# AutonomousVehicleLaboratory/vision_semantic_segmentation

Measured on AMD Instinct MI355X. Metric: fused frames/sec/GPU (1920x1080 + 120k pts) + max|dlog-odds| vs ref, higher is better.
Workload: dtype f16 hi+lo split, MX-FP4 correction passes, fp32 accumulate

## Files before the change

### vision_semantic_segmentation_amd/csrc/seg_gemm.hip

```cpp
#include <cstdlib>
#include <cstring>
#include <type_traits>

#include "seg_types.h"

namespace avl {
namespace {

struct GemmArgs {
    const void* A;
    const void* W;
    const float* bias;
    const void* R;
    void* C;
    int lda, ldr, ldc;
    int M, N, K;
    int relu, out_f32;
    int ntiles;
    int nsub;
    long long a_lo_delta;
    const void* R_lo;
    void* C_lo;
};

// ... 429 lines not shown
                    Vec8<H>::store(cp + 8, hi);
                    if constexpr (IO != 0) {
                        if (csplit) {
#pragma unroll
                            for (int i = 0; i < 8; ++i) { lo[i] = v[i] - (float)(H)v[i]; hi[i] = v[8 + i] - (float)(H)v[8 + i]; }
                            H* cl = c_lo + (long long)m * ldc + cbase;
                            Vec8<H>::store(cl, lo);
                            Vec8<H>::store(cl + 8, hi);
                        }
                    }
                }
            }
        }
        if (t + nwg < total) init_acc(t + nwg);
    }
}

template <typename H, int WM, int WN, int MI, int STAGES, int NSUB, int IO, int AST, bool EXT>
int launch_ring_t(const GemmArgs& a0, int M, hipStream_t s, const RingExt& x) {
    constexpr int BM = WM * MI * 16, BN = WN * 64, LDS = (AST * BM + STAGES * BN) * 128;
    static_assert(LDS <= 160 * 1024, "ring does not fit LDS");
    AVL_HIP_CHECK(hipFuncSetAttribute(reinterpret_cast<const void*>(&k_gemm_ring<H, WM, WN, MI, STAGES, NSUB, IO, AST, EXT>),
                                      hipFuncAttributeMaxDynamicSharedMemorySize, LDS));
    GemmArgs a = a0;
    a.ntiles = (a.N + BN - 1) / BN;
    const int mtiles = (M + BM - 1) / BM;
    const int total = mtiles * a.ntiles;
    const int grid = total < 256 ? total : 256;
    hipLaunchKernelGGL((k_gemm_ring<H, WM, WN, MI, STAGES, NSUB, IO, AST, EXT>), dim3(grid), dim3(WM * WN * 64), LDS, s, a, mtiles, x);
    AVL_LAUNCH_CHECK();
    return AVL_OK;
}

template <typename H, int WM, int WN, int MI, int STAGES, int NSUB = 1, int IO = 0, int AST = STAGES>
int launch_ring(const GemmArgs& a, int M, hipStream_t s, const RingExt* x = nullptr) {
    if (x) return launch_ring_t<H, WM, WN, MI, STAGES, NSUB, IO, AST, true>(a, M, s, *x);
    return launch_ring_t<H, WM, WN, MI, STAGES, NSUB, IO, AST, false>(a, M, s, RingExt{});
}

template <typename T, int WM, int WN>
int launch_cfg(const GemmArgs& a, int mtiles, hipStream_t s) {
    constexpr int LDS = 2 * (WM * 64 + WN * 64) * 128;
    AVL_HIP_CHECK(hipFuncSetAttribute(reinterpret_cast<const void*>(&k_gemm<T, WM, WN>),
                                      hipFuncAttributeMaxDynamicSharedMemorySize, LDS));
    hipLaunchKernelGGL((k_gemm<T, WM, WN>), dim3(mtiles * a.ntiles), dim3(WM * WN * 64), LDS, s, a);
    AVL_LAUNCH_CHECK();
    return AVL_OK;
}

struct MxArgs {
    GemmArgs g;
    const char* Aq[2];
    const char* As[2];
    const char* Wq[2];
    const char* Ws[2];
    int ldaq;
    long long a_srows, w_srows;
    char* Cq[2];
    char* Cs[2];
    int ldcq;
    long long c_srows;
    int nmx;
    const char* Rq;
    const char* Rs;
    int ldrq;
    long long r_srows;
    int nmb1;
    const void* A2;
    int lda2, ldaq2;
    const char* Aq2[2];
    const char* As2[2];
    long long a_srows2;
    int stagger;
};

template <int IO, int MI>
__device__ __forceinline__ void mx_epilogue(const MxArgs& q, f32x4 (&acc)[MI][4], int nt, int mt, int wm, int wn, int fr, int kq) {
    typedef f16 H;
    typedef typename Half16<H>::v8 v8;
    constexpr int BM = 2 * MI * 16, BN = 256;
    const GemmArgs& p = q.g;
    const int nbase = nt * BN + wn * 64 + kq * 16;
    const bool ncol_ok = nbase + 16 <= p.N;
    const bool rsplit = p.R_lo != nullptr, csplit = p.C_lo != nullptr;
    const unsigned m0 = (unsigned)(mt * BM + wm * (MI * 16) + fr);
    const unsigned sc_r = (unsigned)(nbase >> 8) * (unsigned)q.r_srows * 8u + (unsigned)((nbase >> 5) & 7);
    const unsigned sc_c = (unsigned)(nbase >> 8) * (unsigned)q.c_srows * 8u + (unsigned)((nbase >> 5) & 7);
    v8 nr0 = {}, nr1 = {};
    uint2 npk = make_uint2(0u, 0u);
    unsigned nsb = 127u;
    auto load_res = [&](int mi) {
        const unsigned m = m0 + mi * 16;
        if (p.R && (int)m < p.M && ncol_ok) {
            const H* rp = static_cast<const H*>(p.R) + (m * (unsigned)p.ldr + (unsigned)nbase);
            nr0 = *reinterpret_cast<const v8*>(rp);
            nr1 = *reinterpret_cast<const v8*>(rp + 8);
            if (q.Rq) {
                npk = *reinterpret_cast<const uint2*>(q.Rq + (m * (unsigned)q.ldrq + (unsigned)(nbase / 2)));
                nsb = (unsigned char)q.Rs[sc_r + m * 8u];
            }
        }
    };
    load_res(0);
#pragma unroll
    for (int mi = 0; mi < MI; ++mi) {
        const unsigned m = m0 + mi * 16;
        const bool live = (int)m < p.M && ncol_ok;
        const v8 r0 = nr0, r1 = nr1;
        const uint2 pk = npk;
        const unsigned sb = nsb;
        if (mi + 1 < MI) load_res(mi + 1);
        float v[16];
#pragma unroll
        for (int nj = 0; nj < 4; ++nj)
#pragma unroll
            for (int r = 0; r < 4; ++r) v[nj * 4 + r] = acc[mi][nj][r];
        if (p.R && live) {
            float rl[16];
#pragma unroll
            for (int i = 0; i < 16; ++i) rl[i] = 0.f;
            if (rsplit) {
                const H* rlp = static_cast<const H*>(p.R_lo) + (m * (unsigned)p.ldr + (unsigned)nbase);
                const v8 l0 = *reinterpret_cast<const v8*>(rlp), l1 = *reinterpret_cast<const v8*>(rlp + 8);
#pragma unroll
                for (int i = 0; i < 8; ++i) { rl[i] = (float)l0[i]; rl[8 + i] = (float)l1[i]; }
            } else if (q.Rq) {
                typedef float v2f __attribute__((ext_vector_type(2)));
                const float sc = __uint_as_float(sb << 23);
#define AVL_FP4_DEC(w, sel, o) { const v2f d = __builtin_amdgcn_cvt_scalef32_pk_f32_fp4(w, sc, sel); rl[o] = d.x; rl[o + 1] = d.y; }
                AVL_FP4_DEC(pk.x, 0, 0) AVL_FP4_DEC(pk.x, 1, 2) AVL_FP4_DEC(pk.x, 2, 4) AVL_FP4_DEC(pk.x, 3, 6)
                AVL_FP4_DEC(pk.y, 0, 8) AVL_FP4_DEC(pk.y, 1, 10) AVL_FP4_DEC(pk.y, 2, 12) AVL_FP4_DEC(pk.y, 3, 14)
#undef AVL_FP4_DEC
            }
#pragma unroll
            for (int i = 0; i < 8; ++i) { v[i] += (float)r0[i] + rl[i]; v[8 + i] += (float)r1[i] + rl[8 + i]; }
        }
        if (p.relu) {
#pragma unroll
            for (int i = 0; i < 16; ++i) v[i] = fmaxf(v[i], 0.f);
        }
        v8 h0, h1;
#pragma unroll
        for (int i = 0; i < 8; ++i) { h0[i] = (H)v[i]; h1[i] = (H)v[8 + i]; }
        float hi[16], lo[16];
#pragma unroll
        for (int i = 0; i < 8; ++i) {
            hi[i] = (float)h0[i];
            hi[8 + i] = (float)h1[i];
            lo[i] = v[i] - hi[i];
            lo[8 + i] = v[8 + i] - hi[8 + i];
        }
        const unsigned coff = m * (unsigned)p.ldc + (unsigned)nbase;
        if (live) {
            H* cp = static_cast<H*>(p.C) + coff;
            *reinterpret_cast<v8*>(cp) = h0;
            *reinterpret_cast<v8*>(cp + 8) = h1;
        }
        if (csplit) {
            v8 l0, l1;
#pragma unroll
            for (int i = 0; i < 8; ++i) { l0[i] = (H)lo[i]; l1[i] = (H)lo[8 + i]; }
            if (live) {
                H* cl = static_cast<H*>(p.C_lo) + coff;
                *reinterpret_cast<v8*>(cl) = l0;
                *reinterpret_cast<v8*>(cl + 8) = l1;
            }
#pragma unroll
            for (int i = 0; i < 8; ++i) { lo[i] = (float)l0[i]; lo[8 + i] = (float)l1[i]; }
        }
        if constexpr (IO != 0) {
#pragma unroll
            for (int pl = 0; pl < 2; ++pl) {
                if (q.Cq[pl] == nullptr) continue;
                unsigned pq[2];
                const unsigned sq = quantize_fp4_block(pl == 0 ? hi : lo, pq);
                if (live) {
                    *reinterpret_cast<uint2*>(q.Cq[pl] + (m * (unsigned)q.ldcq + (unsigned)(nbase / 2))) = make_uint2(pq[0], pq[1]);
                    if ((kq & 1) == 0) q.Cs[pl][sc_c + m * 8u] = (char)sq;
                }
            }
        }
    }
}

template <int IO, int MI>
__global__ void __launch_bounds__(512) k_gemm_ring_mx(MxArgs q, int mtiles) {
    typedef f16 H;
    typedef typename Half16<H>::v8 v8;
    typedef int v8i __attribute__((ext_vector_type(8)));
    constexpr int WM = 2, WN = 4, STAGES = 2;
    constexpr int NW = WM * WN, BM = WM * MI * 16, BN = WN * 64;
    constexpr int A_BYTES = BM * 128, W_BYTES = BN * 128;
    constexpr int W_REGION = STAGES * A_BYTES, S_REGION = W_REGION + STAGES * W_BYTES;
    constexpr int S_BYTES = 4096;
    constexpr int A_INSTR = BM / 8 / NW, W_INSTR = BN / 8 / NW;
    extern __shared__ __attribute__((aligned(16))) char lds[];
    const GemmArgs& p = q.g;

    const int tid = threadIdx.x, lane = tid & 63;
    const int wave = __builtin_amdgcn_readfirstlane(tid >> 6);
    const int wm = wave / WN, wn = wave % WN;
    const int nwg = gridDim.x;
    int vb;
    {
        const int bid = blockIdx.x, xcd = bid & 7, local = bid >> 3, qq = nwg >> 3, r = nwg & 7;
        vb = (xcd < r ? xcd * (qq + 1) : r * (qq + 1) + (xcd - r) * qq) + local;
    }
    const int total = mtiles * p.ntiles;
    const int nmb = p.K / 256;
    const int nsub = 4 + q.nmx;
    const unsigned lds_base = lds_addr(lds);

    const int srow = lane >> 3, schunk = lane & 7;
    const unsigned ct = (unsigned)((schunk ^ srow) << 4);
    const unsigned a_lane16 = (unsigned)srow * (unsigned)(p.lda * 2) + ct, a_laneq = (unsigned)srow * (unsigned)q.ldaq + ct;
    const unsigned a_lane16_2 = (unsigned)srow * (unsigned)(q.lda2 * 2) + ct, a_laneq_2 = (unsigned)srow * (unsigned)q.ldaq2 + ct;
    unsigned w_off16[W_INSTR], w_offq[W_INSTR];
#pragma unroll
    for (int i = 0; i < W_INSTR; ++i) {
        const int r = (i * NW + wave) * 8 + srow;
        const int key = ((r >> 1) & 1) | (((r >> 4) & 3) << 1);
        w_off16[i] = (unsigned)r * (unsigned)(p.K * 2) + ((schunk ^ key) << 4);
        w_offq[i] = (unsigned)r * (unsigned)(p.K / 2) + ((schunk ^ key) << 4);
    }
    int pt = vb, pmb = 0, pj = 0, issued = 0;
    auto issue = [&]() {
        const int nt = pt % p.ntiles, mt = pt / p.ntiles;
        const unsigned abase = lds_base + (issued % STAGES) * A_BYTES + wave * 1024;
        const unsigned wbase = lds_base + W_REGION + (issued % STAGES) * W_BYTES + wave * 1024;
        const bool second = pmb >= q.nmb1;
        const int mbl = second ? pmb - q.nmb1 : pmb;
        if (pj < 4) {
            const long long rowb = second ? (long long)q.lda2 * 2 : (long long)p.lda * 2;
            const char* sa = static_cast<const char*>(second ? q.A2 : p.A) + ((long long)mt * BM + wave * 8) * rowb + (long long)(mbl * 4 + pj) * 128;
            const char* sw = static_cast<const char*>(p.W) + (long long)nt * BN * p.K * 2 + (long long)(pmb * 4 + pj) * 128;
            const unsigned al = second ? a_lane16_2 : a_lane16;
#pragma unroll
            for (int i = 0; i < A_INSTR; ++i) glds16_saddr(sa + (long long)i * (NW * 8) * rowb, al, abase + i * NW * 1024);
#pragma unroll
            for (int i = 0; i < W_INSTR; ++i) glds16_saddr(sw, w_off16[i], wbase + i * NW * 1024);
        } else {
            const int t = pj - 4;
            const long long rowb = second ? q.ldaq2 : q.ldaq;
            const char* sa = (second ? q.Aq2[t] : q.Aq[t]) + ((long long)mt * BM + wave * 8) * rowb + (long long)mbl * 128;
            const char* sw = q.Wq[t] + (long long)nt * BN * (p.K / 2) + (long long)pmb * 128;
            const unsigned al = second ? a_laneq_2 : a_laneq;
#pragma unroll
            for (int i = 0; i < A_INSTR; ++i) glds16_saddr(sa + (long long)i * (NW * 8) * rowb, al, abase + i * NW * 1024);
#pragma unroll
            for (int i = 0; i < W_INSTR; ++i) glds16_saddr(sw, w_offq[i], wbase + i * NW * 1024);
            if (wave < 4 && (wave >= 2 || wave * 128 < BM)) {
                const char* as = second ? q.As2[t] + ((long long)mbl * q.a_srows2 + (long long)mt * BM) * 8
                                        : q.As[t] + ((long long)mbl * q.a_srows + (long long)mt * BM) * 8;
                const char* ss = wave < 2 ? as + wave * 1024
                                          : q.Ws[t] + ((long long)pmb * q.w_srows + (long long)nt * BN) * 8 + (wave - 2) * 1024;
                glds16_saddr(ss, (unsigned)lane * 16u, lds_base + S_REGION + (issued % STAGES) * S_BYTES + wave * 1024);
// ... 58 lines not shown
                }
            }
            for (int u = 0; u < q.nmx; ++u, ++g) {
                asm volatile("s_waitcnt vmcnt(0)" ::: "memory");
                __builtin_amdgcn_s_barrier();
                const char* abase = lds + (g % STAGES) * A_BYTES + a_row0 * 128;
                const char* wbase = lds + (g % STAGES) * W_BYTES;
                const char* sbase = lds + (g % STAGES) * S_BYTES + S_REGION;
#pragma unroll
                for (int kk = 0; kk < 2; ++kk) {
                    if (kk == late && pt < total) issue();
                    int4 wf[4];
                    int ws[4];
#pragma unroll
                    for (int nj = 0; nj < 4; ++nj) {
                        wf[nj] = *reinterpret_cast<const int4*>(wbase + w_off[nj] + (((kk * 4 + kq) ^ w_key[nj]) << 4));
                        {
                            const uint2 w8 = *reinterpret_cast<const uint2*>(sbase + 2048 + (wn * 4 + (fr >> 2)) * 128 + ((fr & 3) * 4 + kq) * 8);
                            ws[nj] = (int)(((nj < 2 ? w8.x : w8.y) >> (8 * ((nj & 1) * 2 + kk))) & 0xffu);
                        }
                    }
                    const int achunk = ((kk * 4 + kq) ^ a_key) << 4;
                    int4 af = *reinterpret_cast<const int4*>(abase + achunk);
                    unsigned asw = *reinterpret_cast<const unsigned*>(sbase + a_row0 * 8 + kk * 4);
#pragma unroll
                    for (int mi = 0; mi < MI; ++mi) {
                        const int4 cur = af;
                        const int as = (int)((asw >> (8 * kq)) & 0xffu);
                        if (mi + 1 < MI) {
                            af = *reinterpret_cast<const int4*>(abase + (mi + 1) * 2048 + achunk);
                            asw = *reinterpret_cast<const unsigned*>(sbase + (a_row0 + (mi + 1) * 16) * 8 + kk * 4);
                        }
                        const v8i xa = {cur.x, cur.y, cur.z, cur.w, 0, 0, 0, 0};
#pragma unroll
                        for (int nj = 0; nj < 4; ++nj) {
                            const v8i wa = {wf[nj].x, wf[nj].y, wf[nj].z, wf[nj].w, 0, 0, 0, 0};
                            acc[mi][nj] = __builtin_amdgcn_mfma_scale_f32_16x16x128_f8f6f4(wa, xa, acc[mi][nj], 4, 4, 0, ws[nj], 0, as);
                        }
                    }
                }
            }
        }
        mx_epilogue<IO, MI>(q, acc, nt, mt, wm, wn, fr, kq);
        if (t + nwg < total) init_acc(t + nwg);
    }
}

template <int IO, int MI, int LATE>
__global__ void __launch_bounds__(512) k_gemm_mx_pipe(MxArgs q, int mtiles) {
    typedef f16 H;
    typedef typename Half16<H>::v8 v8;
    typedef int v8i __attribute__((ext_vector_type(8)));
    constexpr int WM = 2, WN = 4, STAGES = 2;
    constexpr int NW = WM * WN, BM = WM * MI * 16, BN = WN * 64;
    constexpr int A_BYTES = BM * 128, W_BYTES = BN * 128;
    constexpr int W_REGION = STAGES * A_BYTES, S_REGION = W_REGION + STAGES * W_BYTES;
    constexpr int S_BYTES = 4096;
    constexpr int A_INSTR = BM / 8 / NW, W_INSTR = BN / 8 / NW;
    constexpr int NS = 2 * MI, D = 3, EV = NS - D;
    constexpr int EW = MI == 8 ? 5 : EV;
    extern __shared__ __attribute__((aligned(16))) char lds[];
    const GemmArgs& p = q.g;

    const int tid = threadIdx.x, lane = tid & 63;
    const int wave = __builtin_amdgcn_readfirstlane(tid >> 6);
    const int wm = wave / WN, wn = wave % WN;
    const int nwg = gridDim.x;
    int vb;
    {
        const int bid = blockIdx.x, xcd = bid & 7, local = bid >> 3, qq = nwg >> 3, r = nwg & 7;
        vb = (xcd < r ? xcd * (qq + 1) : r * (qq + 1) + (xcd - r) * qq) + local;
    }
    const int ntiles = p.ntiles, nmx = q.nmx;
    const int total = mtiles * ntiles;
    const int nmb = p.K / 256;
    const int nsub = 4 + nmx;
    const unsigned lds_base = lds_addr(lds);

    auto lane_now = [&]() __attribute__((always_inline)) {
        unsigned l;
        asm volatile("v_mbcnt_lo_u32_b32 %0, -1, 0\n\tv_mbcnt_hi_u32_b32 %0, -1, %0" : "=v"(l));
        return l;
    };
    int pt = vb, pmb = 0, pj = 0, issued = 0, pmbl = 0;
    long long cur_rowb16 = 0, cur_rowbq = 0, cur_asrows = 0;
    const char *cur_a16 = nullptr, *cur_aq = nullptr, *cur_as = nullptr, *cur_w16 = nullptr, *cur_wq = nullptr, *cur_ws = nullptr;
    long long cur_aps = 0, cur_wps = 0;
    int p_mt = 0;
    auto set_input = [&](bool second) __attribute__((always_inline)) {
        const long long rows0 = (long long)p_mt * BM + wave * 8;
        if (!second) {
            cur_rowb16 = (long long)p.lda * 2; cur_rowbq = q.ldaq; cur_asrows = q.a_srows;
            cur_a16 = static_cast<const char*>(p.A) + rows0 * cur_rowb16;
            cur_aq = q.Aq[0] + rows0 * cur_rowbq;
            cur_as = q.As[0] + (long long)p_mt * BM * 8;
            cur_aps = q.Aq[1] - q.Aq[0];
        } else {
            cur_rowb16 = (long long)q.lda2 * 2; cur_rowbq = q.ldaq2; cur_asrows = q.a_srows2;
            cur_a16 = static_cast<const char*>(q.A2) + rows0 * cur_rowb16;
            cur_aq = q.Aq2[0] + rows0 * cur_rowbq;
            cur_as = q.As2[0] + (long long)p_mt * BM * 8;
            cur_aps = q.Aq2[1] - q.Aq2[0];
        }
        pmbl = 0;
    };
    auto set_tile = [&]() __attribute__((always_inline)) {
        const int nt_ = pt % ntiles;
        p_mt = pt / ntiles;
        cur_w16 = static_cast<const char*>(p.W) + (long long)nt_ * BN * p.K * 2;
        cur_wq = q.Wq[0] + (long long)nt_ * BN * (p.K / 2);
        cur_ws = q.Ws[0] + (long long)nt_ * BN * 8;
        cur_wps = q.Wq[1] - q.Wq[0];
        set_input(false);
    };
    auto issue_w = [&]() __attribute__((always_inline)) {
        const unsigned wbase = lds_base + W_REGION + (issued & 1) * W_BYTES + wave * 1024;
        const unsigned l = lane_now(), srow = l >> 3, cw = ((l & 7u) ^ (((srow >> 1) & 1u) | (((unsigned)(wave >> 1) & 3u) << 1))) << 4;
        const unsigned wr0 = (unsigned)wave * 8u + srow;
        if (pj < 4) {
            const char* sw = cur_w16 + (long long)(pmb * 4 + pj) * 128;
            const unsigned wl = wr0 * (unsigned)(p.K * 2) + cw;
#pragma unroll
            for (int i = 0; i < W_INSTR; ++i)
                glds16_saddr(sw + (long long)i * (NW * 8) * p.K * 2, wl, wbase + i * NW * 1024);
        } else {
            const char* sw = cur_wq + (pj == 4 ? 0 : cur_wps) + (long long)pmb * 128;
            const unsigned wl = wr0 * (unsigned)(p.K / 2) + cw;
#pragma unroll
            for (int i = 0; i < W_INSTR; ++i)
                glds16_saddr(sw + (long long)i * (NW * 8) * (p.K / 2), wl, wbase + i * NW * 1024);
        }
    };
    auto issue_a = [&]() __attribute__((always_inline)) {
        const unsigned abase = lds_base + (issued & 1) * A_BYTES + wave * 1024;
        const unsigned l = lane_now(), srow = l >> 3, ct = ((l & 7u) ^ srow) << 4;
        if (pj < 4) {
            const char* sa = cur_a16 + (long long)(pmbl * 4 + pj) * 128;
            const unsigned al = srow * (unsigned)cur_rowb16 + ct;
#pragma unroll
            for (int i = 0; i < A_INSTR; ++i)
                glds16_saddr(sa + (long long)i * (NW * 8) * cur_rowb16, al, abase + i * NW * 1024);
        } else {
            const long long ta = pj == 4 ? 0 : cur_aps, tw = pj == 4 ? 0 : cur_wps;
            const char* sa = cur_aq + ta + (long long)pmbl * 128;
            const unsigned a_lq = srow * (unsigned)cur_rowbq + ct;
#pragma unroll
            for (int i = 0; i < A_INSTR; ++i)
                glds16_saddr(sa + (long long)i * (NW * 8) * cur_rowbq, a_lq, abase + i * NW * 1024);
            if (wave < 4 && (wave >= 2 || wave * 128 < BM)) {
                const char* ss = wave < 2 ? cur_as + ta + (long long)pmbl * cur_asrows * 8 + wave * 1024
                                          : cur_ws + tw + (long long)pmb * q.w_srows * 8 + (wave - 2) * 1024;
                glds16_saddr(ss, l * 16u, lds_base + S_REGION + (issued & 1) * S_BYTES + wave * 1024);
            }
        }
        ++issued;
        if (++pj == nsub) {
            pj = 0;
            ++pmbl;
            if (++pmb == nmb) {
                pmb = 0;
                pt += nwg;
                if (pt < total) set_tile();
            } else if (pmb == q.nmb1) set_input(true);
        }
    };
    if (pt < total) set_tile();
    static_assert(NW == 8, "the DMA stagger assumes waves w and w + 4 on one SIMD");
    const bool early = wave >= 4 || q.stagger == 0;
    if (pt < total) { issue_w(); issue_a(); }
    if (pt < total) { issue_w(); issue_a(); }

    const int fr = lane & 15, kq = lane >> 4;
    const int a_row0 = wm * (MI * 16) + fr;
    const int wrow0 = wn * 64 + (fr >> 2) * 16 + (fr & 3);
    const int wkey_r = ((wrow0 >> 1) & 1) | (((wrow0 >> 4) & 3) << 1);
    const unsigned a_v0 = (unsigned)(a_row0 * 128 + ((kq ^ (a_row0 & 7)) << 4));
    const unsigned w_v0 = (unsigned)(W_REGION + wrow0 * 128 + ((kq ^ wkey_r) << 4));
    const unsigned sa_v = (unsigned)(S_REGION + a_row0 * 8 + kq);
    const unsigned sw_v = (unsigned)(S_REGION + 2048 + (wn * 4 + (fr >> 2)) * 128 + ((fr & 3) * 4 + kq) * 8);

    f32x4 acc[MI][4];
    auto init_acc = [&](int t) {
        const int nb = (t % ntiles) * BN + wn * 64 + kq * 16;
#pragma unroll
        for (int nj = 0; nj < 4; ++nj) {
            const float4 b = *reinterpret_cast<const float4*>(p.bias + nb + 4 * nj);
#pragma unroll
            for (int mi = 0; mi < MI; ++mi) acc[mi][nj] = f32x4{b.x, b.y, b.z, b.w};
        }
    };
    if (vb < total) init_acc(vb);

    int4 Af[NS], Wf[2][4];
    unsigned As[NS];
    uint2 Wsc = make_uint2(0u, 0u), Wsn = make_uint2(0u, 0u);
    auto rdA = [&](const char* slot, int kk, int mi) { return *reinterpret_cast<const int4*>(slot + (a_v0 ^ (unsigned)(kk * 64)) + mi * 2048); };
    auto rdW = [&](const char* slot, int kk, int nj) { return *reinterpret_cast<const int4*>(slot + (w_v0 ^ (unsigned)(kk * 64)) + nj * 512); };
    auto rdAs = [&](const char* slot, int kk, int mi) { return (unsigned)*reinterpret_cast<const unsigned char*>(slot + sa_v + mi * 128 + kk * 4); };
    auto rdWs = [&](const char* slot) { return *reinterpret_cast<const uint2*>(slot + sw_v); };

    int g = 0;
    bool w_sent = false;
    auto step = [&](auto kind_c, auto s_c, const bool next_q) __attribute__((always_inline)) {
        constexpr int KIND = decltype(kind_c)::value, S = decltype(s_c)::value;
        constexpr int kk = S / MI, mi = S % MI;
        const char* ab = lds + (g & 1) * A_BYTES;
        const char* wb = lds + (g & 1) * W_BYTES;
        const char* sb = lds + (g & 1) * S_BYTES;
        const char* abn = lds + ((g + 1) & 1) * A_BYTES;
        const char* wbn = lds + ((g + 1) & 1) * W_BYTES;
        const char* sbn = lds + ((g + 1) & 1) * S_BYTES;
        auto readA = [&](int t) {
            Af[t] = rdA(ab, t / MI, t % MI);
            if (KIND == 1) As[t] = rdAs(sb, t / MI, t % MI);
        };
        auto readAn = [&](int t) {
            Af[t] = rdA(abn, t / MI, t % MI);
            As[t] = rdAs(sbn, t / MI, t % MI);
        };
        if (EW != EV && S == EW) {
            if (LATE == 0 && !early && g > 0 && pt < total) issue_a();
            if (KIND == 0) asm volatile("s_waitcnt lgkmcnt(1)\n\ts_barrier" ::: "memory");
            else asm volatile("s_waitcnt lgkmcnt(2)\n\ts_barrier" ::: "memory");
            __builtin_amdgcn_sched_barrier(0);
            if (early && pt < total) { issue_w(); w_sent = true; }
        }
        if (EW != EV && LATE != 0 && !early && S == EW + LATE && pt < total) {
            issue_w();
            w_sent = true;
        }
        if (S == EV) {
            if (EW != EV && LATE == 0 && !early && pt < total) {
                issue_w();
                w_sent = true;
            }
            if (EW != EV && w_sent) asm volatile("s_waitcnt vmcnt(%0)\n\ts_waitcnt lgkmcnt(0)\n\ts_barrier" ::"n"(W_INSTR) : "memory");
            else asm volatile("s_waitcnt vmcnt(0)\n\ts_waitcnt lgkmcnt(0)\n\ts_barrier" ::: "memory");
            w_sent = false;
            __builtin_amdgcn_sched_barrier(0);
            if (early && pt < total) { if (EW == EV) issue_w(); issue_a(); }
#pragma unroll
            for (int nj = 0; nj < 4; ++nj) Wf[0][nj] = rdW(wbn, 0, nj);
            Wsn = rdWs(sbn);
            readAn(0);
        }
        if (!early && (EW == EV || LATE != 0) && S == EV + LATE && pt < total) {
            if (EW == EV) issue_w();
            issue_a();
        }
        if (S + D < NS) readA(S + D);
        if (S >= EV && S + 1 < NS) readAn(S - EV + 1);
        if constexpr (MI == 8 && S < 4) Wf[1][S] = rdW(wb, 1, S);
        if constexpr (MI == 4 && S < 2) { Wf[1][2 * S] = rdW(wb, 1, 2 * S); Wf[1][2 * S + 1] = rdW(wb, 1, 2 * S + 1); }
        if (KIND == 0) {
            const v8 af = __builtin_bit_cast(v8, Af[S]);
#pragma unroll
            for (int nj = 0; nj < 4; ++nj) acc[mi][nj] = Half16<H>::mfma(__builtin_bit_cast(v8, Wf[kk][nj]), af, acc[mi][nj]);
        } else {
            const v8i xa = {Af[S].x, Af[S].y, Af[S].z, Af[S].w, 0, 0, 0, 0};
            const int as = (int)As[S];
#define AVL_QMFMA(NJ)                                                                                                              \
    do {                                                                                                                           \
        const v8i wa = {Wf[kk][NJ].x, Wf[kk][NJ].y, Wf[kk][NJ].z, Wf[kk][NJ].w, 0, 0, 0, 0};                                       \
        const int ws = (int)((NJ) < 2 ? Wsc.x : Wsc.y);                                                                            \
        acc[mi][NJ] = __builtin_amdgcn_mfma_scale_f32_16x16x128_f8f6f4(wa, xa, acc[mi][NJ], 4, 4, ((NJ) & 1) * 2 + kk, ws, 0, as);      \
    } while (0)
            AVL_QMFMA(0); AVL_QMFMA(1); AVL_QMFMA(2); AVL_QMFMA(3);
#undef AVL_QMFMA
        }
        __builtin_amdgcn_sched_barrier(0);
    };
    auto substep = [&](auto kind_c, const bool next_q) __attribute__((always_inline)) {
#define AVL_STEP(N) step(kind_c, std::integral_constant<int, N>(), next_q)
        AVL_STEP(0); AVL_STEP(1); AVL_STEP(2); AVL_STEP(3); AVL_STEP(4); AVL_STEP(5); AVL_STEP(6); AVL_STEP(7);
        if constexpr (NS == 16) { AVL_STEP(8); AVL_STEP(9); AVL_STEP(10); AVL_STEP(11); AVL_STEP(12); AVL_STEP(13); AVL_STEP(14); AVL_STEP(15); }
#undef AVL_STEP
        Wsc = Wsn;
        ++g;
    };
    typedef std::integral_constant<int, 0> F16;
    typedef std::integral_constant<int, 1> FP4;

    asm volatile("s_waitcnt vmcnt(0)" ::: "memory");
    __builtin_amdgcn_s_barrier();
    for (int t = vb; t < total; t += nwg) {
        const int nt = t % ntiles, mt = t / ntiles;
        {
            const char* ab = lds + (g & 1) * A_BYTES;
            const char* wb = lds + (g & 1) * W_BYTES;
#pragma unroll
            for (int nj = 0; nj < 4; ++nj) Wf[0][nj] = rdW(wb, 0, nj);
#pragma unroll
            for (int s = 0; s < D; ++s) Af[s] = rdA(ab, 0, s);
        }
        for (int mb = 0; mb < nmb; ++mb) {
            for (int j = 0; j < 4; ++j) substep(F16(), j == 3);
            for (int u = 0; u < nmx; ++u) substep(FP4(), u + 1 < nmx);
        }
        mx_epilogue<IO, MI>(q, acc, nt, mt, wm, wn, fr, kq);
        if (t + nwg < total) init_acc(t + nwg);
    }
}

template <int IO, int MI>
int launch_ring_mx_t(const MxArgs& a0, hipStream_t s) {
    constexpr int BM = 2 * MI * 16, LDS = 2 * (BM + 256) * 128 + 2 * 4096;
    MxArgs a = a0;
    a.stagger = 1;
    a.g.ntiles = a.g.N / 256;
    const int mtiles = (a.g.M + BM - 1) / BM;
    const int total = mtiles * a.g.ntiles;
    const int grid = total < 256 ? total : 256;
    if (a.g.K >= 1024) {
        constexpr int LATE = MI == 8 ? 0 : 1;
        AVL_HIP_CHECK(hipFuncSetAttribute(reinterpret_cast<const void*>(&k_gemm_mx_pipe<IO, MI, LATE>), hipFuncAttributeMaxDynamicSharedMemorySize, LDS));
        hipLaunchKernelGGL((k_gemm_mx_pipe<IO, MI, LATE>), dim3(grid), dim3(512), LDS, s, a, mtiles);
    } else {
        AVL_HIP_CHECK(hipFuncSetAttribute(reinterpret_cast<const void*>(&k_gemm_ring_mx<IO, MI>), hipFuncAttributeMaxDynamicSharedMemorySize, LDS));
        hipLaunchKernelGGL((k_gemm_ring_mx<IO, MI>), dim3(grid), dim3(512), LDS, s, a, mtiles);
    }
    AVL_LAUNCH_CHECK();
    return AVL_OK;
}

int launch_ring_mx(const MxArgs& a, int m_image, bool quantize_out, hipStream_t s) {
    const long long t256 = (long long)((m_image + 255) / 256) * (a.g.N / 256);
    const bool small = t256 < 192 || (t256 > 256 && t256 < 384);
    if (small) return quantize_out ? launch_ring_mx_t<1, 4>(a, s) : launch_ring_mx_t<0, 4>(a, s);
    return quantize_out ? launch_ring_mx_t<1, 8>(a, s) : launch_ring_mx_t<0, 8>(a, s);
}

struct TileCfg { int bm, bn; };
inline TileCfg pick_tile(const avl_seg_op& op);
inline bool ring_eligible(const avl_seg_op& op) {
    const int M = op.out_h * op.out_w * op_batch(op);
    return is_half(op.dtype) && op.w_layout != 1 && op.out_c > 64 && !op.out_f32 && op.out_c % 128 == 0 && op.in_rows >= (M + 255) / 256 * 256;
}
inline TileCfg pick_tile(const avl_seg_op& op) {
    if (op.out_c <= 64) return {256, 64};
    return {128, 128};
}
inline int ring_variant(const avl_seg_op& op) {
    const bool can256 = op.out_c % 256 == 0 && op.w_rows % 256 == 0;
    const int m_image = op.out_h * op.out_w;
    int v = op.w_layout;
    if (v == 0) v = (can256 && ((m_image + 255) / 256) * (op.out_c / 256) >= 192) ? 3 : 2;
    if (v == 3 && !can256) v = 2;
    return v;
}
inline bool ring_ext(const avl_seg_op& op) { return op.stride > 1 || op.out2 != nullptr || op.out2_lo != nullptr || op.n_split != 0; }

}

static avl_seg_op gemm_image_op(const avl_seg_op& op, int n) {
    avl_seg_op v = op;
    const long long m = (long long)op.out_h * op.out_w * n;
    const int es = elem_size(op.dtype), oes = op.out_f32 ? 4 : es;
    auto at = [](const void* p, long long bytes) -> const void* { return p ? static_cast<const char*>(p) + bytes : p; };
    v.in = at(op.in, m * op.in_ld * es);
    v.in_lo = at(op.in_lo, m * op.in_ld * es);
    v.in2 = at(op.in2, m * op.in2_ld * es);
    v.in2_lo = at(op.in2_lo, m * op.in2_ld * es);
    v.out = const_cast<void*>(at(op.out, m * op.out_ld * oes));
    v.out_lo = const_cast<void*>(at(op.out_lo, m * op.out_ld * es));
    if (op.out_f32) v.out_mx = const_cast<void*>(at(op.out_mx, m));
    v.bias = op.bias + (long long)n * op.w_rows;
    v.in_rows = (int)(op.in_rows - m);
    v.out_rows = (int)(op.out_rows - m);
    v.batch = 1;
    v.bias_per_image = 0;
    return v;
}

int validate_gemm(const avl_seg_op& op) {
    const int es = elem_size(op.dtype);
    AVL_REQUIRE(is_half(op.dtype) || op.dtype == AVL_F32, "GEMM dtype %d", op.dtype);
    AVL_REQUIRE(op.in && op.out && op.weight && op.bias, "GEMM has NULL buffers");
    AVL_REQUIRE(op.w_layout >= 0 && op.w_layout <= 4, "GEMM w_layout %d (0 = by shape, 1 .. 4 = a forced 16-bit tile configuration)", op.w_layout);
    AVL_REQUIRE(op.w_layout == 0 || is_half(op.dtype), "GEMM w_layout %d forces a tile configuration of the 16-bit kernels: dtype %d", op.w_layout, op.dtype);
    if (op.bias_per_image && op_batch(op) > 1) {
        AVL_REQUIRE(op.w_split != 2 && !op.in3, "GEMM: a per-image bias is not supported by the MX GEMM");
        AVL_REQUIRE(!ring_ext(op), "GEMM: a per-image bias goes with neither strided input rows (stride %d) nor a second destination", op.stride);
        for (int n = 0; n < op.batch; ++n) {
            const avl_seg_op v = gemm_image_op(op, n);
            AVL_REQUIRE(v.in_rows >= (op.out_h * op.out_w + 255) / 256 * 256,
                        "GEMM with a per-image bias: image %d has %d input rows behind its first (the last image needs whole 256-row tiles)", n, v.in_rows);
            const int rc = validate_gemm(v);
            if (rc) return rc;
        }
        return AVL_OK;
    }
    const int M = op.out_h * op.out_w * op_batch(op), K = op.in_c, N = op.out_c;
    AVL_REQUIRE(M > 0 && N > 0 && K > 0, "GEMM M/N/K = %d/%d/%d", M, N, K);
    if (ring_ext(op)) {
        AVL_REQUIRE(op.w_split != 2 && !op.in3, "GEMM: the MX GEMM takes neither strided input rows (stride %d) nor a second destination", op.stride);
        AVL_REQUIRE(is_half(op.dtype) && !op.out_f32, "GEMM: strided input rows (stride %d) / a second destination need a 16-bit GEMM (dtype %d, out_f32 %d)",
                    op.stride, op.dtype, op.out_f32);
// ... 166 lines not shown
```

### vision_semantic_segmentation_amd/csrc/seg_types.h

```cpp
#pragma once
#include <hip/hip_runtime.h>

#include "avl_common.h"

namespace avl {

typedef __bf16 bf16;
typedef __bf16 bf16x8 __attribute__((ext_vector_type(8)));
typedef _Float16 f16;
typedef _Float16 f16x8 __attribute__((ext_vector_type(8)));
typedef float f32x4 __attribute__((ext_vector_type(4)));
typedef float f32x8 __attribute__((ext_vector_type(8)));

template <typename T>
struct Vec8;

template <>
struct Vec8<bf16> {
    static __device__ __forceinline__ void load(const bf16* p, float (&v)[8]) {
        const bf16x8 x = *reinterpret_cast<const bf16x8*>(p);
#pragma unroll
        for (int i = 0; i < 8; ++i) v[i] = (float)x[i];
    }
    static __device__ __forceinline__ void store(bf16* p, const float (&v)[8]) {
// ... 3 lines not shown
        *reinterpret_cast<bf16x8*>(p) = x;
    }
};

template <>
struct Vec8<f16> {
    static __device__ __forceinline__ void load(const f16* p, float (&v)[8]) {
        const f16x8 x = *reinterpret_cast<const f16x8*>(p);
#pragma unroll
        for (int i = 0; i < 8; ++i) v[i] = (float)x[i];
    }
    static __device__ __forceinline__ void store(f16* p, const float (&v)[8]) {
        f16x8 x;
#pragma unroll
        for (int i = 0; i < 8; ++i) x[i] = (f16)v[i];
        *reinterpret_cast<f16x8*>(p) = x;
    }
};

template <typename H>
struct Half16;
template <>
struct Half16<bf16> {
    typedef bf16x8 v8;
    static __device__ __forceinline__ f32x4 mfma(v8 a, v8 b, f32x4 c) { return __builtin_amdgcn_mfma_f32_16x16x32_bf16(a, b, c, 0, 0, 0); }
    static __device__ __forceinline__ float dot2(uint32_t a, uint32_t b, float c) {
        typedef __bf16 v2 __attribute__((ext_vector_type(2)));
        return __builtin_amdgcn_fdot2_f32_bf16(__builtin_bit_cast(v2, a), __builtin_bit_cast(v2, b), c, false);
    }
};
template <>
struct Half16<f16> {
    typedef f16x8 v8;
    static __device__ __forceinline__ f32x4 mfma(v8 a, v8 b, f32x4 c) { return __builtin_amdgcn_mfma_f32_16x16x32_f16(a, b, c, 0, 0, 0); }
    static __device__ __forceinline__ float dot2(uint32_t a, uint32_t b, float c) {
        typedef _Float16 v2 __attribute__((ext_vector_type(2)));
        return __builtin_amdgcn_fdot2(__builtin_bit_cast(v2, a), __builtin_bit_cast(v2, b), c, false);
    }
};

template <>
struct Vec8<float> {
    static __device__ __forceinline__ void load(const float* p, float (&v)[8]) {
        const float4 a = *reinterpret_cast<const float4*>(p);
        const float4 b = *reinterpret_cast<const float4*>(p + 4);
        v[0] = a.x; v[1] = a.y; v[2] = a.z; v[3] = a.w;
        v[4] = b.x; v[5] = b.y; v[6] = b.z; v[7] = b.w;
    }
    static __device__ __forceinline__ void store(float* p, const float (&v)[8]) {
        *reinterpret_cast<float4*>(p) = make_float4(v[0], v[1], v[2], v[3]);
        *reinterpret_cast<float4*>(p + 4) = make_float4(v[4], v[5], v[6], v[7]);
    }
};

template <typename T>
__device__ __forceinline__ float to_f32(T v) { return (float)v; }
template <typename T>
__device__ __forceinline__ T from_f32(float v) { return (T)v; }

__device__ __forceinline__ void glds16_asm(const void* g, unsigned lds_byte_addr) {
    unsigned keep;
    asm volatile(
        "s_mov_b32 %0, m0\n\t"
        "s_mov_b32 m0, %2\n\t"
        "s_nop 0\n\t"
        "global_load_lds_dwordx4 %1, off\n\t"
        "s_mov_b32 m0, %0"
        : "=&s"(keep)
        : "v"(g), "s"(lds_byte_addr)
        : "memory");
}

__device__ __forceinline__ void glds16_saddr(const void* sbase, unsigned voff, unsigned lds_byte_addr) {
    unsigned keep;
    asm volatile(
        "s_mov_b32 %0, m0\n\t"
        "s_mov_b32 m0, %3\n\t"
        "s_nop 0\n\t"
        "global_load_lds_dwordx4 %1, %2\n\t"
        "s_mov_b32 m0, %0"
        : "=&s"(keep)
        : "v"(voff), "s"(sbase), "s"(lds_byte_addr)
        : "memory");
}

__device__ __forceinline__ void glds4_saddr(const void* sbase, unsigned voff, unsigned lds_byte_addr) {
    unsigned keep;
    asm volatile(
        "s_mov_b32 %0, m0\n\t"
        "s_mov_b32 m0, %3\n\t"
        "s_nop 0\n\t"
        "global_load_lds_dword %1, %2\n\t"
        "s_mov_b32 m0, %0"
        : "=&s"(keep)
        : "v"(voff), "s"(sbase), "s"(lds_byte_addr)
        : "memory");
}

__device__ __forceinline__ unsigned mx_fp4_scale_byte(float amax) {
    const unsigned ab = __float_as_uint(amax), e = ab >> 23;
    return (e >= 3u ? e - 2u : 1u) + ((ab & 0x7fffffu) > 0x500000u ? 1u : 0u);
}

__device__ __forceinline__ unsigned quantize_fp4_block(const float (&v)[16], unsigned (&q)[2]) {
    float amax = 0.f;
#pragma unroll
    for (int i = 0; i < 16; ++i) amax = fmaxf(amax, fabsf(v[i]));
    {
        const unsigned ab = __float_as_uint(amax);
        const auto r16 = __builtin_amdgcn_permlane16_swap(ab, ab, false, false);
        amax = __uint_as_float(max(r16[0], r16[1]));
    }
    const unsigned sbyte = mx_fp4_scale_byte(amax);
    const float scale = __uint_as_float(sbyte << 23);
    q[0] = q[1] = 0u;
#define AVL_FP4_PAIR(i)                                                                                  \
    q[0] = __builtin_amdgcn_cvt_scalef32_pk_fp4_f32(q[0], v[2 * (i)], v[2 * (i) + 1], scale, (i));        \
    q[1] = __builtin_amdgcn_cvt_scalef32_pk_fp4_f32(q[1], v[8 + 2 * (i)], v[8 + 2 * (i) + 1], scale, (i))
    AVL_FP4_PAIR(0); AVL_FP4_PAIR(1); AVL_FP4_PAIR(2); AVL_FP4_PAIR(3);
#undef AVL_FP4_PAIR
    return sbyte;
}

__device__ __forceinline__ unsigned lds_addr(const void* p) {
    return (unsigned)(size_t)(const __attribute__((address_space(3))) void*)p;
}

inline int elem_size(int dtype) { return dtype == AVL_F32 ? 4 : 2; }

inline int op_batch(const avl_seg_op& op) { return op.batch > 1 ? op.batch : 1; }
template <typename T>
__device__ __forceinline__ T* image_base(T* p, long long pixels, long long ld) {
    return p ? p + (long long)blockIdx.z * pixels * ld : p;
}
inline bool is_half(int dtype) { return dtype == AVL_BF16 || dtype == AVL_F16; }

template <typename C>
struct MxBundle {
    C* q[2];
    C* s[2];
    int ldq;
    long long srows;
};
template <typename C>
inline MxBundle<C> mx_bundle_at(C* b, long long rows, long long channels) {
    const long long P = rows * (channels / 2), S = (channels / 256) * rows * 8;
    return {{b, b + P + S}, {b + P, b + 2 * P + S}, (int)(channels / 2), rows};
}
inline MxBundle<char> mx_bundle(void* base, long long rows, long long channels) { return mx_bundle_at(static_cast<char*>(base), rows, channels); }
inline MxBundle<const char> mx_bundle(const void* base, long long rows, long long channels) { return mx_bundle_at(static_cast<const char*>(base), rows, channels); }

int launch_gemm(const avl_seg_op& op, hipStream_t s);
int validate_gemm(const avl_seg_op& op);
int launch_conv_op(const avl_seg_op& op, hipStream_t s);
int validate_conv_op(const avl_seg_op& op);
int launch_gconv_mfma(const avl_seg_op& op, hipStream_t s);
int validate_gconv_mfma(const avl_seg_op& op);
int launch_conv3x3(const avl_seg_op& op, hipStream_t s);
int validate_conv3x3(const avl_seg_op& op);
int launch_stem_mfma(const avl_seg_op& op, hipStream_t s);
int launch_stem_pre_f32(const avl_seg_op& op, hipStream_t s);
int launch_dwconv_k(const avl_seg_op& op, hipStream_t s);
int validate_dwconv_k(const avl_seg_op& op);
int launch_dwpw(const avl_seg_op& op, hipStream_t s);
int validate_dwpw(const avl_seg_op& op);
int launch_bottleneck(const avl_seg_op& op, hipStream_t s);
int validate_bottleneck(const avl_seg_op& op);

}
```

Measured before the change: 212.5.

## Cut SGPR pressure in MX GEMM pipe by deriving bundle offsets and running pointers

Reworks address generation in the MX FP4 pipelined GEMM. Per-input strides and plane offsets are now derived from K and the row counts, which the host checks with new bundle-layout assertions. Walking pointers are advanced incrementally instead of being recomputed from 64-bit base plus offset. Kernel arguments are re-read from the kernarg segment around the epilogue, the epilogue flags are packed into one scalar word, and a new load helper no longer saves and restores m0. The aim is to lower scalar register pressure and address-arithmetic overhead in the issue loop. In exchange, inputs must use the dense bundle layout and offsets are narrowed to 32 bits.

```diff
diff --git a/vision_semantic_segmentation_amd/csrc/seg_gemm.hip b/vision_semantic_segmentation_amd/csrc/seg_gemm.hip
--- a/vision_semantic_segmentation_amd/csrc/seg_gemm.hip
+++ b/vision_semantic_segmentation_amd/csrc/seg_gemm.hip
@@ -535,7 +535,10 @@
     const GemmArgs& p = q.g;
     const int nbase = nt * BN + wn * 64 + kq * 16;
     const bool ncol_ok = nbase + 16 <= p.N;
-    const bool rsplit = p.R_lo != nullptr, csplit = p.C_lo != nullptr;
+    enum { F_RES = 1, F_RES_LO16 = 2, F_RES_LOQ = 4, F_OUT_LO16 = 8, F_RELU = 16, F_OUT_Q0 = 32, F_OUT_Q1 = 64 };
+    unsigned fl = (p.R ? F_RES : 0) | (p.R_lo ? F_RES_LO16 : 0) | (q.Rq ? F_RES_LOQ : 0) | (p.C_lo ? F_OUT_LO16 : 0) | (p.relu ? F_RELU : 0) |
+                  (q.Cq[0] ? F_OUT_Q0 : 0) | (q.Cq[1] ? F_OUT_Q1 : 0);
+    asm volatile("" : "+s"(fl));
     const unsigned m0 = (unsigned)(mt * BM + wm * (MI * 16) + fr);
     const unsigned sc_r = (unsigned)(nbase >> 8) * (unsigned)q.r_srows * 8u + (unsigned)((nbase >> 5) & 7);
     const unsigned sc_c = (unsigned)(nbase >> 8) * (unsigned)q.c_srows * 8u + (unsigned)((nbase >> 5) & 7);
@@ -544,11 +547,11 @@
     unsigned nsb = 127u;
     auto load_res = [&](int mi) {
         const unsigned m = m0 + mi * 16;
-        if (p.R && (int)m < p.M && ncol_ok) {
-            const H* rp = static_cast<const H*>(p.R) + (m * (unsigned)p.ldr + (unsigned)nbase);
+        if ((fl & F_RES) && (int)m < p.M && ncol_ok) {
+            const H* rp = reinterpret_cast<const H*>(static_cast<const char*>(p.R) + (m * (unsigned)p.ldr + (unsigned)nbase) * 2u);
             nr0 = *reinterpret_cast<const v8*>(rp);
             nr1 = *reinterpret_cast<const v8*>(rp + 8);
-            if (q.Rq) {
+            if (fl & F_RES_LOQ) {
                 npk = *reinterpret_cast<const uint2*>(q.Rq + (m * (unsigned)q.ldrq + (unsigned)(nbase / 2)));
                 nsb = (unsigned char)q.Rs[sc_r + m * 8u];
             }
@@ -568,16 +571,16 @@
         for (int nj = 0; nj < 4; ++nj)
 #pragma unroll
             for (int r = 0; r < 4; ++r) v[nj * 4 + r] = acc[mi][nj][r];
-        if (p.R && live) {
+        if ((fl & F_RES) && live) {
             float rl[16];
 #pragma unroll
             for (int i = 0; i < 16; ++i) rl[i] = 0.f;
-            if (rsplit) {
-                const H* rlp = static_cast<const H*>(p.R_lo) + (m * (unsigned)p.ldr + (unsigned)nbase);
+            if (fl & F_RES_LO16) {
+                const H* rlp = reinterpret_cast<const H*>(static_cast<const char*>(p.R_lo) + (m * (unsigned)p.ldr + (unsigned)nbase) * 2u);
                 const v8 l0 = *reinterpret_cast<const v8*>(rlp), l1 = *reinterpret_cast<const v8*>(rlp + 8);
 #pragma unroll
                 for (int i = 0; i < 8; ++i) { rl[i] = (float)l0[i]; rl[8 + i] = (float)l1[i]; }
-            } else if (q.Rq) {
+            } else if (fl & F_RES_LOQ) {
                 typedef float v2f __attribute__((ext_vector_type(2)));
                 const float sc = __uint_as_float(sb << 23);
 #define AVL_FP4_DEC(w, sel, o) { const v2f d = __builtin_amdgcn_cvt_scalef32_pk_f32_fp4(w, sc, sel); rl[o] = d.x; rl[o + 1] = d.y; }
@@ -588,7 +591,7 @@
 #pragma unroll
             for (int i = 0; i < 8; ++i) { v[i] += (float)r0[i] + rl[i]; v[8 + i] += (float)r1[i] + rl[8 + i]; }
         }
-        if (p.relu) {
+        if (fl & F_RELU) {
 #pragma unroll
             for (int i = 0; i < 16; ++i) v[i] = fmaxf(v[i], 0.f);
         }
@@ -603,18 +606,18 @@
             lo[i] = v[i] - hi[i];
             lo[8 + i] = v[8 + i] - hi[8 + i];
         }
-        const unsigned coff = m * (unsigned)p.ldc + (unsigned)nbase;
+        const unsigned coff = (m * (unsigned)p.ldc + (unsigned)nbase) * 2u;
         if (live) {
-            H* cp = static_cast<H*>(p.C) + coff;
+            H* cp = reinterpret_cast<H*>(static_cast<char*>(p.C) + coff);
             *reinterpret_cast<v8*>(cp) = h0;
             *reinterpret_cast<v8*>(cp + 8) = h1;
         }
-        if (csplit) {
+        if (fl & F_OUT_LO16) {
             v8 l0, l1;
 #pragma unroll
             for (int i = 0; i < 8; ++i) { l0[i] = (H)lo[i]; l1[i] = (H)lo[8 + i]; }
             if (live) {
-                H* cl = static_cast<H*>(p.C_lo) + coff;
+                H* cl = reinterpret_cast<H*>(static_cast<char*>(p.C_lo) + coff);
                 *reinterpret_cast<v8*>(cl) = l0;
                 *reinterpret_cast<v8*>(cl + 8) = l1;
             }
@@ -624,7 +627,7 @@
         if constexpr (IO != 0) {
 #pragma unroll
             for (int pl = 0; pl < 2; ++pl) {
-                if (q.Cq[pl] == nullptr) continue;
+                if (!(fl & (pl == 0 ? F_OUT_Q0 : F_OUT_Q1))) continue;
                 unsigned pq[2];
                 const unsigned sq = quantize_fp4_block(pl == 0 ? hi : lo, pq);
                 if (live) {
@@ -849,35 +852,45 @@
         asm volatile("v_mbcnt_lo_u32_b32 %0, -1, 0\n\tv_mbcnt_hi_u32_b32 %0, -1, %0" : "=v"(l));
         return l;
     };
-    int pt = vb, pmb = 0, pj = 0, issued = 0, pmbl = 0;
-    long long cur_rowb16 = 0, cur_rowbq = 0, cur_asrows = 0;
-    const char *cur_a16 = nullptr, *cur_aq = nullptr, *cur_as = nullptr, *cur_w16 = nullptr, *cur_wq = nullptr, *cur_ws = nullptr;
-    long long cur_aps = 0, cur_wps = 0;
+    int pt = vb, pmb = 0, pj = 0, issued = 0;
+    unsigned cur_rowb16 = 0;
+    const char *run_a16 = nullptr, *run_aq = nullptr, *run_as = nullptr, *run_w16 = nullptr, *run_wq = nullptr, *run_ws = nullptr;
+    unsigned cur_aps = 0;
+    const char *c_A, *c_A2, *c_Aq, *c_Aq2, *c_W, *c_Wq;
+    unsigned K, K1, arows, wrows;
+    unsigned asb, wsb;
+    unsigned w_pb, wps;
+    auto read_args = [&]() __attribute__((always_inline)) {
+        auto ka = __builtin_amdgcn_kernarg_segment_ptr();
+        asm volatile("" : "+s"(ka));
+        const MxArgs* a = (const MxArgs*)ka;
+        c_A = static_cast<const char*>(a->g.A); c_A2 = static_cast<const char*>(a->A2); c_Aq = a->Aq[0]; c_Aq2 = a->Aq2[0];
+        c_W = static_cast<const char*>(a->g.W); c_Wq = a->Wq[0];
+        K = (unsigned)a->g.K; K1 = (unsigned)a->nmb1 * 256u; arows = (unsigned)a->a_srows; wrows = (unsigned)a->w_srows;
+        asm volatile("" : "+s"(c_A), "+s"(c_A2), "+s"(c_Aq), "+s"(c_Aq2), "+s"(c_W), "+s"(c_Wq), "+s"(K), "+s"(K1), "+s"(arows), "+s"(wrows));
+        asb = arows * 8u; wsb = wrows * 8u;
+        w_pb = (unsigned)mx_plane_bytes(wrows, K); wps = w_pb + (unsigned)mx_scale_bytes(wrows, K);
+    };
+    read_args();
     int p_mt = 0;
     auto set_input = [&](bool second) __attribute__((always_inline)) {
         const long long rows0 = (long long)p_mt * BM + wave * 8;
-        if (!second) {
-            cur_rowb16 = (long long)p.lda * 2; cur_rowbq = q.ldaq; cur_asrows = q.a_srows;
-            cur_a16 = static_cast<const char*>(p.A) + rows0 * cur_rowb16;
-            cur_aq = q.Aq[0] + rows0 * cur_rowbq;
-            cur_as = q.As[0] + (long long)p_mt * BM * 8;
-            cur_aps = q.Aq[1] - q.Aq[0];
-        } else {
-            cur_rowb16 = (long long)q.lda2 * 2; cur_rowbq = q.ldaq2; cur_asrows = q.a_srows2;
-            cur_a16 = static_cast<const char*>(q.A2) + rows0 * cur_rowb16;
-            cur_aq = q.Aq2[0] + rows0 * cur_rowbq;
-            cur_as = q.As2[0] + (long long)p_mt * BM * 8;
-            cur_aps = q.Aq2[1] - q.Aq2[0];
-        }
-        pmbl = 0;
+        const unsigned kin = second ? K - K1 : K1;
+        const char* a16 = second ? c_A2 : c_A;
+        const char* aq = second ? c_Aq2 : c_Aq;
+        const unsigned a_pb = (unsigned)mx_plane_bytes(arows, kin);
+        cur_rowb16 = kin * 2u;
+        run_a16 = a16 + rows0 * cur_rowb16;
+        run_aq = aq + rows0 * (kin / 2u);
+        run_as = aq + a_pb + (unsigned)(p_mt * BM * 8);
+        cur_aps = a_pb + (unsigned)mx_scale_bytes(arows, kin);
     };
     auto set_tile = [&]() __attribute__((always_inline)) {
         const int nt_ = pt % ntiles;
         p_mt = pt / ntiles;
-        cur_w16 = static_cast<const char*>(p.W) + (long long)nt_ * BN * p.K * 2;
-        cur_wq = q.Wq[0] + (long long)nt_ * BN * (p.K / 2);
-        cur_ws = q.Ws[0] + (long long)nt_ * BN * 8;
-        cur_wps = q.Wq[1] - q.Wq[0];
+        run_w16 = c_W + (long long)nt_ * BN * K * 2;
+        run_wq = c_Wq + (long long)nt_ * BN * (K / 2u);
+        run_ws = c_Wq + w_pb + (unsigned)(nt_ * BN * 8);
         set_input(false);
     };
     auto issue_w = [&]() __attribute__((always_inline)) {
@@ -885,50 +898,52 @@
         const unsigned l = lane_now(), srow = l >> 3, cw = ((l & 7u) ^ (((srow >> 1) & 1u) | (((unsigned)(wave >> 1) & 3u) << 1))) << 4;
         const unsigned wr0 = (unsigned)wave * 8u + srow;
         if (pj < 4) {
-            const char* sw = cur_w16 + (long long)(pmb * 4 + pj) * 128;
-            const unsigned wl = wr0 * (unsigned)(p.K * 2) + cw;
-#pragma unroll
-            for (int i = 0; i < W_INSTR; ++i)
-                glds16_saddr(sw + (long long)i * (NW * 8) * p.K * 2, wl, wbase + i * NW * 1024);
+            const char* sw = run_w16;
+            const unsigned rb = K * 2u, wl = wr0 * rb + cw;
+#pragma unroll
+            for (int i = 0; i < W_INSTR; ++i, sw += rb * (NW * 8))
+                glds16_saddr_m0(sw, wl, wbase + i * NW * 1024);
         } else {
-            const char* sw = cur_wq + (pj == 4 ? 0 : cur_wps) + (long long)pmb * 128;
-            const unsigned wl = wr0 * (unsigned)(p.K / 2) + cw;
-#pragma unroll
-            for (int i = 0; i < W_INSTR; ++i)
-                glds16_saddr(sw + (long long)i * (NW * 8) * (p.K / 2), wl, wbase + i * NW * 1024);
+            const char* sw = run_wq + (pj == 4 ? 0u : wps);
+            const unsigned rb = K / 2u, wl = wr0 * rb + cw;
+#pragma unroll
+            for (int i = 0; i < W_INSTR; ++i, sw += rb * (NW * 8))
+                glds16_saddr_m0(sw, wl, wbase + i * NW * 1024);
         }
     };
     auto issue_a = [&]() __attribute__((always_inline)) {
         const unsigned abase = lds_base + (issued & 1) * A_BYTES + wave * 1024;
         const unsigned l = lane_now(), srow = l >> 3, ct = ((l & 7u) ^ srow) << 4;
         if (pj < 4) {
-            const char* sa = cur_a16 + (long long)(pmbl * 4 + pj) * 128;
-            const unsigned al = srow * (unsigned)cur_rowb16 + ct;
-#pragma unroll
-            for (int i = 0; i < A_INSTR; ++i)
-                glds16_saddr(sa + (long long)i * (NW * 8) * cur_rowb16, al, abase + i * NW * 1024);
+            const char* sa = run_a16;
+            const unsigned al = srow * cur_rowb16 + ct;
+#pragma unroll
+            for (int i = 0; i < A_INSTR; ++i, sa += cur_rowb16 * (NW * 8))
+                glds16_saddr_m0(sa, al, abase + i * NW * 1024);
+            run_a16 += 128;
+            run_w16 += 128;
         } else {
-            const long long ta = pj == 4 ? 0 : cur_aps, tw = pj == 4 ? 0 : cur_wps;
-            const char* sa = cur_aq + ta + (long long)pmbl * 128;
-            const unsigned a_lq = srow * (unsigned)cur_rowbq + ct;
-#pragma unroll
-            for (int i = 0; i < A_INSTR; ++i)
-                glds16_saddr(sa + (long long)i * (NW * 8) * cur_rowbq, a_lq, abase + i * NW * 1024);
+            const unsigned ta = pj == 4 ? 0u : cur_aps, tw = pj == 4 ? 0u : wps;
+            const char* sa = run_aq + ta;
+            const unsigned cur_rowbq = cur_rowb16 >> 2, a_lq = srow * cur_rowbq + ct;
+#pragma unroll
+            for (int i = 0; i < A_INSTR; ++i, sa += cur_rowbq * (NW * 8))
+                glds16_saddr_m0(sa, a_lq, abase + i * NW * 1024);
             if (wave < 4 && (wave >= 2 || wave * 128 < BM)) {
-                const char* ss = wave < 2 ? cur_as + ta + (long long)pmbl * cur_asrows * 8 + wave * 1024
-                                          : cur_ws + tw + (long long)pmb * q.w_srows * 8 + (wave - 2) * 1024;
-                glds16_saddr(ss, l * 16u, lds_base + S_REGION + (issued & 1) * S_BYTES + wave * 1024);
+                const char* ss = wave < 2 ? run_as + ta + wave * 1024 : run_ws + tw + (wave - 2) * 1024;
+                glds16_saddr_m0(ss, l * 16u, lds_base + S_REGION + (issued & 1) * S_BYTES + wave * 1024);
             }
         }
         ++issued;
         if (++pj == nsub) {
             pj = 0;
-            ++pmbl;
+            run_aq += 128; run_as += asb;
+            run_wq += 128; run_ws += wsb;
             if (++pmb == nmb) {
                 pmb = 0;
                 pt += nwg;
                 if (pt < total) set_tile();
-            } else if (pmb == q.nmb1) set_input(true);
+            } else if (pmb * 256u == K1) set_input(true);
         }
     };
     if (pt < total) set_tile();
@@ -947,16 +962,16 @@
     const unsigned sw_v = (unsigned)(S_REGION + 2048 + (wn * 4 + (fr >> 2)) * 128 + ((fr & 3) * 4 + kq) * 8);
 
     f32x4 acc[MI][4];
-    auto init_acc = [&](int t) {
+    auto init_acc = [&](const float* bias, int t) {
         const int nb = (t % ntiles) * BN + wn * 64 + kq * 16;
 #pragma unroll
         for (int nj = 0; nj < 4; ++nj) {
-            const float4 b = *reinterpret_cast<const float4*>(p.bias + nb + 4 * nj);
+            const float4 b = *reinterpret_cast<const float4*>(bias + nb + 4 * nj);
 #pragma unroll
             for (int mi = 0; mi < MI; ++mi) acc[mi][nj] = f32x4{b.x, b.y, b.z, b.w};
         }
     };
-    if (vb < total) init_acc(vb);
+    if (vb < total) init_acc(p.bias, vb);
 
     int4 Af[NS], Wf[2][4];
     unsigned As[NS];
@@ -1064,8 +1079,12 @@
             for (int j = 0; j < 4; ++j) substep(F16(), j == 3);
             for (int u = 0; u < nmx; ++u) substep(FP4(), u + 1 < nmx);
         }
-        mx_epilogue<IO, MI>(q, acc, nt, mt, wm, wn, fr, kq);
-        if (t + nwg < total) init_acc(t + nwg);
+        auto ka = __builtin_amdgcn_kernarg_segment_ptr();
+        asm volatile("" : "+s"(ka));
+        const MxArgs qe = *(const MxArgs*)ka;
+        mx_epilogue<IO, MI>(qe, acc, nt, mt, wm, wn, fr, kq);
+        if (t + nwg < total) init_acc(qe.g.bias, t + nwg);
+        read_args();
     }
 }
 
@@ -1080,6 +1099,15 @@
     const int grid = total < 256 ? total : 256;
     if (a.g.K >= 1024) {
         constexpr int LATE = MI == 8 ? 0 : 1;
+        const long long K = a.g.K, K1 = (long long)a.nmb1 * 256, K2 = K - K1;
+        auto bundle_ok = [&](const char* const* bq, const char* const* bs, long long rows, long long ch) {
+            const long long P = mx_plane_bytes(rows, ch), S = mx_scale_bytes(rows, ch);
+            return bs[0] - bq[0] == P && (a.nmx < 2 || (bq[1] - bq[0] == P + S && bs[1] - bq[0] == 2 * P + S)) && 2 * (P + S) < (1LL << 32);
+        };
+        AVL_REQUIRE(a.g.lda == K1 && a.ldaq == K1 / 2 && bundle_ok(a.Aq, a.As, a.a_srows, K1), "MX GEMM: first input is not dense rows + a bundle");
+        AVL_REQUIRE(K2 == 0 || (a.lda2 == K2 && a.ldaq2 == K2 / 2 && a.a_srows2 == a.a_srows && bundle_ok(a.Aq2, a.As2, a.a_srows, K2)),
+                    "MX GEMM: second input is not dense rows + a bundle of the first input's rows");
+        AVL_REQUIRE(bundle_ok(a.Wq, a.Ws, a.w_srows, K), "MX GEMM: weights are not a bundle");
         AVL_HIP_CHECK(hipFuncSetAttribute(reinterpret_cast<const void*>(&k_gemm_mx_pipe<IO, MI, LATE>), hipFuncAttributeMaxDynamicSharedMemorySize, LDS));
         hipLaunchKernelGGL((k_gemm_mx_pipe<IO, MI, LATE>), dim3(grid), dim3(512), LDS, s, a, mtiles);
     } else {
diff --git a/vision_semantic_segmentation_amd/csrc/seg_types.h b/vision_semantic_segmentation_amd/csrc/seg_types.h
--- a/vision_semantic_segmentation_amd/csrc/seg_types.h
+++ b/vision_semantic_segmentation_amd/csrc/seg_types.h
@@ -109,6 +109,16 @@
         : "=&s"(keep)
         : "v"(voff), "s"(sbase), "s"(lds_byte_addr)
         : "memory");
+}
+
+__device__ __forceinline__ void glds16_saddr_m0(const void* sbase, unsigned voff, unsigned lds_byte_addr) {
+    asm volatile(
+        "s_mov_b32 m0, %2\n\t"
+        "s_nop 0\n\t"
+        "global_load_lds_dwordx4 %0, %1"
+        :
+        : "v"(voff), "s"(sbase), "s"(lds_byte_addr)
+        : "memory", "m0");
 }
 
 __device__ __forceinline__ void glds4_saddr(const void* sbase, unsigned voff, unsigned lds_byte_addr) {
@@ -169,9 +179,11 @@
     int ldq;
     long long srows;
 };
+__host__ __device__ inline long long mx_plane_bytes(long long rows, long long channels) { return rows * (channels / 2); }
+__host__ __device__ inline long long mx_scale_bytes(long long rows, long long channels) { return (channels / 256) * rows * 8; }
 template <typename C>
 inline MxBundle<C> mx_bundle_at(C* b, long long rows, long long channels) {
-    const long long P = rows * (channels / 2), S = (channels / 256) * rows * 8;
+    const long long P = mx_plane_bytes(rows, channels), S = mx_scale_bytes(rows, channels);
     return {{b, b + P + S}, {b + P, b + 2 * P + S}, (int)(channels / 2), rows};
 }
 inline MxBundle<char> mx_bundle(void* base, long long rows, long long channels) { return mx_bundle_at(static_cast<char*>(base), rows, channels); }
```

Result: faster. 215.4 (median of 6 runs) (+1.4%).
